# ChristianSteger/HORAYZON

Measured on AMD Instinct MI355X. Metric: grid_cells_per_s (horizon_gridded, 360 azimuths, 3601^2 SRTM-like tile), higher is better.
Workload: dtype f32

## Files before the change

horayzon_amd/csrc/hz_api.hip:

```cpp
#include "hz_internal.h"
#include "hz_horisun_plan.h"
#include "hz_horisun_coarse_plan.h"
#include <cmath>
#include <cstring>
#include <cstdlib>
#include <string>
#include <vector>
#include <limits>
#include <mutex>
#include <utility>
#include <thread>
#include <atomic>

namespace hz {

static thread_local std::string g_error;

int set_error(int code, const char *fmt, ...) {
    char buf[1024];
    va_list ap;
    va_start(ap, fmt);
    vsnprintf(buf, sizeof(buf), fmt, ap);
    va_end(ap);
    g_error = buf;
// ... 644 lines not shown
        const int rb = row_begin + k * chunk_rows, re = std::min(rb + chunk_rows, row_end);
        const void *src = (k & 1) ? tmp_hori2 : tmp_hori;
        Ev &e = evs[ev_of[(size_t)k]];
        char *dst = reinterpret_cast<char *>(hori_row0 + (size_t)rb * dim_in_1 * azim_num);
        const size_t bytes = (size_t)(re - rb) * row_bytes;
        std::vector<size_t> cuts;
        if (!pinner.planned.empty()) cuts = pinner.cuts_for(dst, bytes);
        cuts.push_back(bytes);
        if (hipStreamWaitEvent(st_copy, e.c, 0) != hipSuccess)
            return set_error(HZ_ERR_HIP, "copy of the horizon chunk failed: %s", hipGetErrorString(hipGetLastError()));
        size_t from = 0;
        for (size_t to : cuts) {
            if (to > from && hipMemcpyAsync(dst + from, static_cast<const char *>(src) + from, to - from, hipMemcpyDeviceToHost, st_copy) != hipSuccess)
                return set_error(HZ_ERR_HIP, "copy of the horizon chunk failed: %s", hipGetErrorString(hipGetLastError()));
            from = to;
        }
        if (hipEventRecord(e.d, st_copy) != hipSuccess)
            return set_error(HZ_ERR_HIP, "copy of the horizon chunk failed: %s", hipGetErrorString(hipGetLastError()));
        return HZ_OK;
    };
    auto fail = [&](int code) { (void)hipStreamSynchronize(st); if (st_copy) (void)hipStreamSynchronize(st_copy); free_events(); return code; };
    int n_chunk = 0;
    unsigned long long left_cells = 0, left_again = 0;
    float ms_left = 0.0f;
    for (int rb = row_begin; rb < row_end; rb += chunk_rows, n_chunk++) {
        const int re = std::min(rb + chunk_rows, row_end);
        float *hori_chunk;
        if (stream_out) hori_chunk = (float *)((n_chunk & 1) ? tmp_hori2 : tmp_hori);
        else if (skip_hori || to_planes) hori_chunk = (float *)tmp_hori;
        else hori_chunk = d_hori.dev + (size_t)(rb - row_begin) * dim_in_1 * azim_num;
        a.hori = hori_chunk - (size_t)rb * dim_in_1 * azim_num;
        a.row_begin = rb; a.row_end = re;
        if (use_near) {
            NearArgs na;
            na.vec_norm = norm0; na.vec_north = north0; na.mask = mask0;
            na.azim_sin = d_as.dev; na.azim_cos = d_ac.dev;
            na.offset_0 = offset_0; na.offset_1 = offset_1; na.dim_in_1 = dim_in_1; na.row_begin = rb; na.row_end = re;
            na.azim_num = azim_num; na.elev_num = tb.elev_num;
            na.ray_org_elev = ray_org_elev; na.hori_acc = tb.hori_acc; na.low = tb.low; na.up = tb.up;
            na.reasons = near_reasons;
            na.ignore_bad_map = near_opt < 0 ? 1 : 0;
            if ((rc = near_prepass(sc, na, st, &ms_near))) return fail(rc);
            a.near_idx = na.near_idx; a.near_r = na.near_r;
        }
        {
            Ev e;
// ... 81 lines not shown
                const size_t cc = (size_t)(re - rb) * dim_in_1, c0 = plane_cell0 + (size_t)(rb - row_begin) * dim_in_1;
                if (planes_on_dev) rc = hori_to_planes_launch(hori_chunk, cc, azim_num, hori_planes, plane_stride, c0, st);
                else {
                    rc = hori_to_planes_launch(hori_chunk, cc, azim_num, (float *)tmp_planes, cc, 0, st);
                    if (!rc && hipMemcpy2DAsync(hori_planes + c0, plane_stride * sizeof(float), tmp_planes, cc * sizeof(float),
                                                cc * sizeof(float), (size_t)azim_num, hipMemcpyDeviceToHost, st) != hipSuccess)
                        rc = set_error(HZ_ERR_HIP, "copy of the horizon planes failed: %s", hipGetErrorString(hipGetLastError()));
                }
            }
            if (!rc && stream_out && n_chunk >= 1) rc = copy_out(n_chunk - 1);
            if (rc) return fail(rc);
            unsigned long long c[HZ_CNT_N];
            if (hipMemcpyAsync(c, cnt_dev, sizeof(c), hipMemcpyDeviceToHost, st) != hipSuccess ||
                hipStreamSynchronize(st) != hipSuccess)
                return fail(set_error(HZ_ERR_HIP, "horizon kernel failed: %s", hipGetErrorString(hipGetLastError())));
            float m1 = 0.0f, m2 = 0.0f;
            (void)hipEventElapsedTime(&m1, e.a, e.b);
            (void)hipEventElapsedTime(&m2, e.b, e.c);
            ms += m1; ms_svf += m2;
            if (evs.back().l) { float m3 = 0.0f; (void)hipEventElapsedTime(&m3, evs.back().l, e.b); ms_left += m3; }
            for (int k = 0; k < 16; k++) cnt[k] += c[k];
            left_cells += c[28]; left_again += c[29];
            n_verified += c[21];
            if (a.count_work && opts && opts->verbose >= 3) {
                const unsigned long long t0 = ~c[20];
                fprintf(stderr, "hz xcd spans [ms] rows %d..%d:", rb, re);
                for (int x = 0; x < 8; x++) fprintf(stderr, " %.1f", c[12 + x] ? (double)(c[12 + x] - t0) * 1.0e-5 : 0.0);
                fprintf(stderr, "\n");
            }
        }
    }
    Timer t_d2h; t_d2h.start();
    if (stream_out) {
        rc = copy_out(n_chunk - 1);
        const hipError_t se = hipStreamSynchronize(st_copy);
        pinner.finish();
        if (!rc && se != hipSuccess) rc = set_error(HZ_ERR_HIP, "copy of the horizon failed: %s", hipGetErrorString(se));
        if (rc) { free_events(); return rc; }
    }
    free_events();
    HZ_HIP(hipGetLastError());
    if ((rc = d_hori.finish(st))) return rc;
    if ((rc = d_svf.finish(st))) return rc;
    if ((rc = d_vsf.finish(st))) return rc;
    if ((rc = d_open.finish(st))) return rc;
    HZ_HIP(hipStreamSynchronize(st));
    const double d2h_s = t_d2h.stop();

    if (stats) {
        stats->num_rays += cnt[0]; stats->guard_events += cnt[1];
        stats->nodes_visited += cnt[2]; stats->tris_tested += cnt[3]; stats->num_cells += cnt[4];
        stats->wave_node_iters += cnt[5]; stats->wave_leaf_iters += cnt[6]; stats->wave_refills += cnt[7];
        stats->t_h2d_s += h2d_s; stats->t_kernel_s += (double)ms * 1e-3; stats->t_svf_s += (double)ms_svf * 1e-3;
        stats->t_d2h_s += d2h_s;
        stats->t_total_s += t_total.stop();
        stats->elev_num = tb.elev_num; stats->bvh_height = sc->hdr.height; stats->scene_bytes = sc->hdr.total_bytes;
        stats->stack_fallbacks += (uint64_t)fallbacks; stats->stack_redo_blocks += redo_blocks; stats->left_redo_groups += redo_groups;
        stats->rays_shortened += cnt[9]; stats->near_violations += cnt[10] + n_mon_violations; stats->t_near_s += (double)ms_near * 1e-3;
        stats->guard_cells += cnt[11]; stats->near_verified += n_verified;
        stats->t_left_s += (double)ms_left * 1e-3; stats->left_cells += left_cells; stats->left_again += left_again;
        stats->scratch_bytes = (uint64_t)((use_near ? sc->near_bytes : 0) + (n_left_launches > 0 ? sc->left_bytes : 0) + tmp_bytes);
        stats->height_field = height_field ? 1 : 0; stats->near_used = use_near ? 1 : 0;
    }
    if (near_reasons) print_near_reasons(near_reasons);
    if (opts && opts->verbose)
        print_reference_report(sc, alg, cnt[4], cnt[0], slab_cells, dim_in_0, dim_in_1, azim_num, (double)ms * 1e-3,
                               !use_near && near_opt <= 0 && !height_field && !bad_map, use_near && bad_map);
    return HZ_OK;
}

static int locations_run(const Scene *sc, const float *coords, const float *vec_norm, const float *vec_north,
                         float *hori_buffer, float *hori_dist_buffer, int num_loc, int azim_num,
                         float dist_search, float hori_acc, const char *ray_algorithm, float elev_ang_low_lim,
                         const float *ray_org_elev, int hori_dist_out, const hz_opts *opts, hz_stats *stats) {
    int alg = 1;
    int rc = parse_alg(ray_algorithm, &alg);
    if (rc) return rc;
    if (hori_dist_out && alg == 2)
        return set_error(HZ_ERR_ARG, "horizon detection algorithm 'guess_constant' not implemented for horizon "
                                     "distance computation");
    if (!coords || !vec_norm || !vec_north || !ray_org_elev || !hori_buffer) return set_error(HZ_ERR_ARG, "NULL argument");
    if (hori_dist_out && !hori_dist_buffer) return set_error(HZ_ERR_ARG, "hori_dist_buffer is NULL");
    if (num_loc <= 0 || azim_num <= 0) return set_error(HZ_ERR_ARG, "num_loc and azim_num must be positive");
    if (!(hori_acc > 0.0f) || hori_acc > 10.0f) return set_error(HZ_ERR_ARG, "limit of hori_acc (10 degree) is exceeded");
    HZ_HIP(hipSetDevice(sc->device));
    std::lock_guard<std::mutex> run_lock(sc->run_mu);
    hipStream_t st = sc->stream;
// ... 545 lines not shown
    const size_t bytes = (n ? n : 1) * 4;
    HZ_HIP(hipMalloc(&di, bytes)); HZ_HIP(hipMalloc(&dout, bytes)); HZ_HIP(hipMalloc(&tmp, scan_temp_elems(n) * 4 + 16));
    HZ_HIP(hipMemcpy(di, in, n * 4, hipMemcpyHostToDevice));
    rc = exclusive_scan_u32((const uint32_t *)di, (uint32_t *)dout, n, (uint32_t *)tmp, st);
    if (!rc) {
        HZ_HIP(hipStreamSynchronize(st));
        HZ_HIP(hipMemcpy(out, dout, n * 4, hipMemcpyDeviceToHost));
    }
    (void)hipFree(di); (void)hipFree(dout); (void)hipFree(tmp);
    return rc;
}

int hz_debug_valu_peak(int device, int packed, int waves_per_simd, double *winst_per_s_per_simd,
                       double *clock_ghz, int *simds) {
    int rc = select_device(device);
    if (rc) return rc;
    return bench_valu_peak(packed, waves_per_simd, winst_per_s_per_simd, clock_ghz, simds);
}

int hz_debug_set(const char *key, int value) {
    if (!key) return hz::set_error(HZ_ERR_ARG, "hz_debug_set: null key");
    if (!strcmp(key, "shadow_fast_cap")) hz::g_shadow_fast_cap.store(value < 0 ? HZ_SHADOW_FAST_CAP_DEFAULT : value, std::memory_order_relaxed);
    else if (!strcmp(key, "topo_wide")) hz::g_topo_wide.store(value != 0, std::memory_order_relaxed);
    else if (!strcmp(key, "accum_chunk")) hz::g_accum_chunk.store(value < 0 ? 0 : value, std::memory_order_relaxed);
    else if (!strcmp(key, "coarse_tile")) hz::g_coarse_tile.store(value < 0 ? 0 : value, std::memory_order_relaxed);
    else if (!strcmp(key, "horisun_chunk")) hz::g_horisun_chunk.store(value < 0 ? 0 : value, std::memory_order_relaxed);
    else if (!strcmp(key, "horisun_coarse_tile")) hz::g_horisun_coarse_tile.store(value < 0 ? 0 : value, std::memory_order_relaxed);
    else if (!strcmp(key, "horisun_coarse_route")) hz::g_horisun_coarse_route.store(value < 0 ? -1 : (value == 1 ? 1 : 0), std::memory_order_relaxed);
    else if (!strcmp(key, "planes_chunk")) g_planes_chunk.store(value < 0 ? 0 : value, std::memory_order_relaxed);
    else return hz::set_error(HZ_ERR_ARG, "hz_debug_set: unknown key '%s'", key);
    return HZ_OK;
}

int hz_debug_inst_rate(int device, int op, double *cycles_per_inst) {
    int rc = select_device(device);
    if (rc) return rc;
    return bench_inst_rate(op, cycles_per_inst);
}

int hz_debug_copy_peak(int device, size_t bytes, double *gbs) {
    int rc = select_device(device);
    if (rc) return rc;
    return bench_copy_peak(bytes, gbs);
}

static int slope_api(int which, const float *x, const float *y, const float *z, int len_0, int len_1,
// ... 1085 lines not shown
```

horayzon_amd/csrc/hz_common.h:

```cpp
#pragma once
#include <stdint.h>
#include <hip/hip_runtime.h>

#define HZ_BLOB_MAGIC 0x485a4c42u
#define HZ_BLOB_VERSION 10u
#define HZ_WAVE 64

struct BlobHeader {
    uint32_t magic, version;
    int32_t d0, d1;
    int32_t n_quads, n_tin, n_prims, n_nodes;
    int32_t height, n_top;
    float center[3];
    float pad;
    float lo[3], hi[3];
    uint32_t reserved0[2];
    uint64_t off_verts, off_nodes, off_prims, total_bytes;
    uint64_t off_anc;
    int32_t anc_levels;
    int32_t n_prim_slots;
    uint32_t flags;
    uint32_t n_flipped;
    uint64_t off_bad;
    int32_t bad_nb;
// ... 291 lines not shown
__device__ __forceinline__ void hz_load_node_lds(const float4 *q, float4 &n0, uint4 &n1) {
    const unsigned addr = (unsigned)(size_t)reinterpret_cast<const __attribute__((address_space(3))) char *>(
        (const __attribute__((address_space(3))) float4 *)q);
    asm volatile("ds_read_b128 %0, %2\n\t"
                 "ds_read_b128 %1, %2 offset:16\n\t"
                 "s_waitcnt lgkmcnt(0)"
                 : "=&v"(n0), "=&v"(n1)
                 : "v"(addr)
                 : "memory");
}

__device__ __forceinline__ void hz_load_prim(const Prim *q, float4 &q0, float4 &q1, float4 &q2) {
    asm volatile("global_load_dwordx4 %0, %3, off\n\t"
                 "global_load_dwordx4 %1, %3, off offset:16\n\t"
                 "global_load_dwordx4 %2, %3, off offset:32\n\t"
                 "s_waitcnt vmcnt(0)"
                 : "=&v"(q0), "=&v"(q1), "=&v"(q2)
                 : "v"(q)
                 : "memory");
}

struct TravCounters { unsigned nodes, tris, w_nodes, w_leaves;
};
struct TravState { int node, sp, pf, pm, lq0, lq1; };

__device__ __forceinline__ void hz_trav_reset(TravState &t) {
    t.node = 0; t.sp = 0; t.pf = 0; t.pm = 0; t.lq0 = HZ_EMPTY; t.lq1 = HZ_EMPTY;
}

__device__ __forceinline__ int hz_entry_pack(int pf, int pm) {
    return (int)((unsigned)pf | (((unsigned)pm >> 1) & 3u) | (((unsigned)pm & 8u) << 27));
}
__device__ __forceinline__ void hz_entry_unpack(int e, int &pf, int &pm) {
    pm = (int)((((unsigned)e & 3u) << 1) | (((unsigned)e >> 27) & 8u));
    pf = (int)((unsigned)e & 0xbffffffcu);
}

#define HZ_WAVE_TICK(c, lane_) do { const unsigned long long m_ = __ballot(1); if ((lane_) == __ffsll((long long)m_) - 1) (c)++; } while (0)

template <int TPB, bool COUNT, int QLEN = 2, bool NODELET = false, bool LEVELSTACK = true>
__device__ __forceinline__ int hz_trace(const Node *__restrict__ nodes, const Prim *__restrict__ prims,
                                        const float4 *top, int ntop, int *stack, int tid,
                                        float ox, float oy, float oz, float dx, float dy, float dz, float tfar,
                                        float tfar_box, const RayBox &rb, TravState &t, int regroup, int leaf_bias,
                                        TravCounters &cnt, int stack_cap, bool &overflow) {
    const int lane = tid & 63;
    int node = t.node, sp = t.sp, pf = t.pf, pm = t.pm, lq0 = t.lq0, lq1 = t.lq1;
    const int n_entry = __popcll(__ballot(1));
#define HZ_POP() do { \
        if (LEVELSTACK) { \
            if (pm == 0) { const bool ne = sp > 0; sp = ne ? sp - 1 : 0; const int pv = stack[sp * TPB + tid]; \
                           hz_entry_unpack(ne ? pv : 0, pf, pm); } \
            const int slot_ = __builtin_ctz((unsigned)pm | 16u); \
            node = (pm != 0) ? pf + slot_ : HZ_EMPTY; pm &= pm - 1; \
        } else { \
            node = HZ_STACK_AT(sa + (unsigned)(TPB * 4)); sa -= (unsigned)(TPB * 4); \
        } } while (0)
typedef __attribute__((address_space(3))) int hz_lds_int;
#define HZ_STACK_AT(addr) (*reinterpret_cast<hz_lds_int *>((size_t)(addr)))
#define HZ_SAVE() do { if (!LEVELSTACK) sp = (int)(sa - sa0) / (TPB * 4) + 1; \
                       t.node = node; t.sp = sp; t.pf = pf; t.pm = pm; t.lq0 = lq0; t.lq1 = lq1; } while (0)
    const unsigned sa0 = (unsigned)(size_t)reinterpret_cast<hz_lds_int *>(
                             (__attribute__((address_space(3))) char *)reinterpret_cast<char *>(stack)) + (unsigned)tid * 4u;
    unsigned sa = sa0 + (unsigned)(sp - 1) * (unsigned)(TPB * 4);
    const unsigned sa_cap = sa0 + (unsigned)(stack_cap - 5) * (unsigned)(TPB * 4);
    if (!LEVELSTACK) HZ_STACK_AT(sa0) = HZ_EMPTY;
    unsigned sa_hi = 0u;
    const int n_leave = max(min(regroup, n_entry), 1);
// ... 43 lines not shown
                        if (pm != 0) { stack[sp * TPB + tid] = hz_entry_pack(pf, pm); sp++; }
                        pf = first; pm = h;
                    }
                    HZ_POP();
                } else {
                    int m0, m1, m2, m3;
                    hz_node_hit_masks(nr, rb, tfar_box, n1, m0, m1, m2, m3);
                    sa_hi = max(sa_hi, sa);
                    sa = min(sa, sa_cap);
                    const unsigned S = (unsigned)(TPB * 4);
                    const int pv = HZ_STACK_AT(sa + S);
                    const unsigned a0 = (unsigned)m0 & S, a1 = (unsigned)m1 & S, a2 = (unsigned)m2 & S, a3 = (unsigned)m3 & S;
                    const unsigned o32 = a3 | a2, o321 = o32 | a1, o3210 = o321 | a0;
#define HZ_SEL(m, x, y) (((m) & (x)) | (~(m) & (y)))
                    int next = HZ_SEL(m3, first + 3, pv);
                    HZ_STACK_AT(sa + 2u * S) = next; sa += a2 & a3;   next = HZ_SEL(m2, first + 2, next);
                    HZ_STACK_AT(sa + 2u * S) = next; sa += a1 & o32;  next = HZ_SEL(m1, first + 1, next);
                    HZ_STACK_AT(sa + 2u * S) = next; sa += a0 & o321; next = HZ_SEL(m0, first, next);
#undef HZ_SEL
                    node = next; sa = sa + o3210 - S;
                }
            }
        } else {
            if (can_leaf) {
                float4 q0, q1, q2;
                hz_load_prim(prims + HZ_LEAF_ID(lq0), q0, q1, q2);
                if (COUNT) { cnt.tris += (q2.y == q2.y) ? 2 : 1; HZ_WAVE_TICK(cnt.w_leaves, lane); }
                const bool hit = hz_quad_hit(ox, oy, oz, dx, dy, dz, tfar, q0.x, q0.y, q0.z, q0.w, q1.x, q1.y, q1.z, q1.w,
                                             q2.x, q2.y, q2.z, q2.w, q2.y == q2.y);
                if (hit) { lq0 = HZ_LEAF_ID(lq0); node = HZ_EMPTY; }
                else { lq0 = lq1; lq1 = HZ_EMPTY; }
            }
        }
        top_of_iteration();
    }
    if (!LEVELSTACK && sa_hi > sa_cap) overflow = true;
    const bool blocked = lq0 >= 0 && lq0 != HZ_EMPTY;
    const int res = blocked ? 1 : ((HZ_IS_NODE(node) || lq0 < 0) ? 2 : 0);
    if (blocked) lq0 = (int)((unsigned)lq0 | 0x80000000u);
    HZ_SAVE();
    return res;
#undef HZ_POP
#undef HZ_SAVE
#undef HZ_STACK_AT
}

// ... 43 lines not shown
```

horayzon_amd/csrc/hz_horizon.hip:

```cpp
#include "hz_search.h"
#include <vector>

namespace hz {

#ifndef HZ_TPB
#define HZ_TPB 256
#endif
#define HZ_WPB (HZ_TPB / 64)
#ifndef HZ_QLEN
#define HZ_QLEN 2
#endif

struct HorizonParams {
    SceneView sv;
    Tables tb;
    const float *vec_norm, *vec_north;
    const uint8_t *mask;
    float *hori;
    int offset_0, offset_1, dim_in_1;
    int row_begin, row_end;
    TileMap tm;
    float dist, hori_fill, ray_org_elev;
    float dist_box, neg_tau;
    int top_nodes, regroup, stack_bytes, leaf_bias, stage_bytes, hit_cache, stack_cap;
// ... 5 lines not shown
    unsigned verify_mask;
    unsigned long long *counters;
    const int *tile_list;
    int n_list;
    int *redo_list;
    int left_min, left_mode;
    unsigned left_in_base;
    unsigned left_out_base, left_out_cap;
    unsigned *left_rec, *left_in_ctl, *left_out_ctl;
    const unsigned *left_perm;
    int persist;
    unsigned *queue;
};

__device__ __forceinline__ void hz_left_write(unsigned *w, unsigned cert, unsigned k, unsigned flags,
                                                        unsigned ind, unsigned prev, unsigned pazim, unsigned count, float lim_up, float lim_low,
                                                        float elev_samp, float ev, unsigned cache, float st0, float st1, float st2) {
    w[0] = cert;
    w[1] = k; w[2] = flags; w[3] = ind; w[4] = prev; w[5] = pazim; w[6] = count;
    w[7] = __float_as_uint(lim_up); w[8] = __float_as_uint(lim_low); w[9] = __float_as_uint(elev_samp); w[10] = __float_as_uint(ev);
    w[11] = cache; w[12] = __float_as_uint(st0); w[13] = __float_as_uint(st1); w[14] = __float_as_uint(st2); w[15] = 0u;
}

template <int ALG, bool COUNT, bool STAGE, bool NODELET, bool LEVELSTACK, bool LEFT = false>
#ifndef HZ_WG_PER_CU
#define HZ_WG_PER_CU 5
#endif
__global__ __launch_bounds__(HZ_TPB, (COUNT ? 4 : HZ_WG_PER_CU) * (4 / HZ_WPB)) void k_horizon(HorizonParams p_arg) {
    typedef const __attribute__((address_space(4))) HorizonParams *hz_kparams;
    hz_kparams pk = (hz_kparams)__builtin_amdgcn_kernarg_segment_ptr();
#if defined(__HIP_DEVICE_COMPILE__)
#define HZ_LOAD_PARAMS(dst) dst = *pk
#else
#define HZ_LOAD_PARAMS(dst) dst = p_arg
#endif
    HorizonParams p;
    HZ_LOAD_PARAMS(p);
    extern __shared__ __attribute__((aligned(16))) unsigned char smem[];
    int *stack = reinterpret_cast<int *>(smem + p.pre_bytes);
    const float4 *top = reinterpret_cast<const float4 *>(smem + p.pre_bytes + p.stack_bytes);
    const int tid = threadIdx.x;
    const int ntop = p.top_nodes;
    if (NODELET && ntop > 0) {
        float4 *dst = reinterpret_cast<float4 *>(smem + p.pre_bytes + p.stack_bytes);
        const float4 *src = reinterpret_cast<const float4 *>(p.sv.nodes);
        for (int i = tid; i < ntop * 2; i += HZ_TPB) dst[i] = src[i];
        __syncthreads();
// ... 98 lines not shown
            done = true;
        } else {
            const float norm_x = p.vec_norm[3 * cell], norm_y = p.vec_norm[3 * cell + 1], norm_z = p.vec_norm[3 * cell + 2];
            const float north_x = p.vec_north[3 * cell], north_y = p.vec_north[3 * cell + 1], north_z = p.vec_north[3 * cell + 2];
            const float *v = p.sv.verts + 3 * ((size_t)(i + p.offset_0) * p.sv.d1 + (size_t)(j + p.offset_1));
            ox = v[0] + norm_x * p.ray_org_elev;
            oy = v[1] + norm_y * p.ray_org_elev;
            oz = v[2] + norm_z * p.ray_org_elev;
            r01 = north_x; r02 = norm_x;
            r11 = north_y; r12 = norm_y;
            r21 = north_z; r22 = norm_z;
        }
    }
#define HZ_OC(ocx, ocy, ocz) float ocx, ocy, ocz; { float ax_ = ox, ay_ = oy, az_ = oz; \
        asm volatile("" : "+v"(ax_), "+v"(ay_), "+v"(az_)); \
        ocx = ax_ - p.sv.cx; ocy = ay_ - p.sv.cy; ocz = az_ - p.sv.cz; }
    const float tfar = p.dist;

    Search s;
    s.k = 0; s.phase = PH_NEWAZ; s.ind = 0; s.prev = 0; s.pazim = 0; s.count = 0;
    s.lim_up = 0; s.lim_low = 0; s.elev_samp = 0; s.ev = 0;
    unsigned rays = 0, guards = 0, w_adv = 0;
    TravCounters tc; tc.nodes = 0; tc.tris = 0; tc.w_nodes = 0; tc.w_leaves = 0;
    const unsigned cells_cnt = (in_dom && !done && !LEFT) ? 1u : 0u;
    bool ray_active = false, last_hit = false;
    float dx = 0, dy = 0, dz = 1;
    RayBox rb = hz_raybox(0, 0, 0, 0, 0, 1);
    TravState ts; hz_trav_reset(ts);
    int cache = 0;
    bool second = false;
    bool overflow = false;
    unsigned shortened = 0;
    unsigned w_verified = 0, w_violations = 0;
    bool verifying = false, first_result = false, want_v = false;
    float tn = 0.0f;
    bool had_guard = false;
    if (LEFT && !done) {
        s.k = (int)rec[1]; s.phase = (int)(rec[2] & 0xffu); s.ind = (int)rec[3]; s.prev = (int)rec[4]; s.pazim = (int)rec[5]; s.count = (int)rec[6];
        s.lim_up = __uint_as_float(rec[7]); s.lim_low = __uint_as_float(rec[8]); s.elev_samp = __uint_as_float(rec[9]); s.ev = __uint_as_float(rec[10]);
        cache = (int)rec[11];
        last_hit = (rec[2] & 0x100u) != 0u;
        had_guard = (rec[2] & 0x400u) != 0u;
        if (STAGE) { out.stage[0] = __uint_as_float(rec[12]); out.stage[out.stride] = __uint_as_float(rec[13]); out.stage[2 * out.stride] = __uint_as_float(rec[14]); }
        if (rec[2] & 0x200u) {
            const float ec = t.elev_cos[s.ind], es = t.elev_sin[s.ind];
            const float rx = ec * t.azim_sin[s.k], ry = ec * t.azim_cos[s.k], rz = es;
// ... 59 lines not shown
                dx = (r00 * rx + r01 * ry) + r02 * rz;
                dy = (r10 * rx + r11 * ry) + r12 * rz;
                dz = (r20 * rx + r21 * ry) + r22 * rz;
                    tn = (s.ind >= near_i) ? near_rad : p.neg_tau;
                if (COUNT && tn > 0.0f) shortened++;
                if (COUNT) want_v = p.verify_near && tn > 0.0f && (((rays + cert) & p.verify_mask) == 0u);
                HZ_OC(ocx, ocy, ocz)
                rb = hz_raybox(ocx + tn * dx, ocy + tn * dy, ocz + tn * dz, dx, dy, dz);
                hz_trav_reset(ts);
                second = p.hit_cache && (cache != 0) && (s.ind <= s.pazim) && (s.k > 0);
                if (second) {
                    ts.node = cache;
                    if (!LEVELSTACK) { ts.sp = 1; stack[HZ_TPB + tid] = 0; second = false; }
                }
                ray_active = true;
                rays++;
            } else {
                done = true;
            }
        }
        bool start_v = false, viol = false;
        if (ray_active) {
            int r;
            r = hz_trace<HZ_TPB, COUNT, HZ_QLEN, NODELET, LEVELSTACK>(p.sv.nodes, p.sv.prims, top, ntop, stack, tid, ox, oy, oz,
                                                 dx, dy, dz, tfar, p.dist_box, rb, ts, p.regroup, p.leaf_bias, tc, p.stack_cap, overflow);
            if (r == 0 && second) {
                second = false; hz_trav_reset(ts);
            } else if (COUNT && want_v && r != 2) {
                want_v = false; verifying = true; first_result = (r == 1); start_v = true;
                HZ_OC(ocx, ocy, ocz)
                rb = hz_raybox(ocx + p.neg_tau * dx, ocy + p.neg_tau * dy, ocz + p.neg_tau * dz, dx, dy, dz);
                hz_trav_reset(ts);
            } else if (r != 2) {
                if (COUNT && verifying) { viol = ((r == 1) != first_result); verifying = false; }
                ray_active = false; last_hit = (r == 1);
                if (r == 1) cache = p.sv.anc[HZ_LEAF_ID(ts.lq0)];
            }
        }
        if (COUNT) {
            w_verified += (unsigned)__popcll(__ballot(start_v));
            w_violations += (unsigned)__popcll(__ballot(viol));
        }
    }
    unsigned long long r = rays, g = guards, nc = tc.nodes, tcn = tc.tris, cc = cells_cnt;
    unsigned long long wn = tc.w_nodes, wl = tc.w_leaves, wa = w_adv;
    for (int off = 32; off > 0; off >>= 1) {
        r += __shfl_xor(r, off); g += __shfl_xor(g, off); cc += __shfl_xor(cc, off);
        if (COUNT) {
            nc += __shfl_xor(nc, off); tcn += __shfl_xor(tcn, off);
            wn += __shfl_xor(wn, off); wl += __shfl_xor(wl, off); wa += __shfl_xor(wa, off);
        }
    }
    const bool wave_overflowed = !LEVELSTACK && __ballot(overflow) != 0ull;
    if (wave_overflowed) {
        if (lane == 0) {
            const unsigned long long slot = atomicAdd(&p.counters[LEFT ? 30 : 8], 1ull);
            if (slot < (unsigned long long)HZ_REDO_CAP) p.redo_list[(LEFT ? HZ_REDO_CAP : 0) + (int)slot] = blk;
        }
    } else {
    const int guard_cells = __popcll(__ballot(guards != 0u && !(LEFT && had_guard)));
    if (lane == 0) {
        if (r) atomicAdd(&p.counters[0], r);
        if (g) { atomicAdd(&p.counters[1], g); atomicAdd(&p.counters[11], (unsigned long long)guard_cells); }
        if (cc) atomicAdd(&p.counters[4], cc);
        if (COUNT) {
            atomicAdd(&p.counters[2], nc); atomicAdd(&p.counters[3], tcn);
            atomicAdd(&p.counters[5], wn); atomicAdd(&p.counters[6], wl); atomicAdd(&p.counters[7], wa);
        }
    }
    if (COUNT) {
        if (lane == 0) {
            const unsigned xcc = __builtin_amdgcn_s_getreg((3 << 11) | 20) & 7u;
            atomicMax(&p.counters[12 + xcc], (unsigned long long)wall_clock64());
            atomicMax(&p.counters[20], ~t_start);
        }
    }
    if (COUNT) {
        unsigned long long sh = shortened;
        for (int off = 32; off > 0; off >>= 1) sh += __shfl_xor(sh, off);
        if (lane == 0) {
            if (sh) atomicAdd(&p.counters[9], sh);
            if (w_violations) atomicAdd(&p.counters[10], (unsigned long long)w_violations);
            if (w_verified) atomicAdd(&p.counters[21], (unsigned long long)w_verified);
        }
    }
    }
    if (!p.persist) break;
  }
}

static long long resident_workgroups(const void *func, size_t lds) {
    struct Key { const void *f; size_t lds; int dev; long long n; };
    static std::mutex mu;
    static std::vector<Key> cache;
    int dev = 0;
    if (hipGetDevice(&dev) != hipSuccess) { (void)hipGetLastError(); return 0; }
    std::lock_guard<std::mutex> lock(mu);
    for (const Key &k : cache) if (k.f == func && k.lds == lds && k.dev == dev) return k.n;
    int per_cu = 0;
    hipDeviceProp_t prop;
    long long n = 0;
    if (hipOccupancyMaxActiveBlocksPerMultiprocessor(&per_cu, func, HZ_TPB, lds) == hipSuccess && per_cu > 0 &&
        hipGetDeviceProperties(&prop, dev) == hipSuccess && prop.multiProcessorCount > 0)
        n = (long long)per_cu * prop.multiProcessorCount;
    else (void)hipGetLastError();
    cache.push_back(Key{func, lds, dev, n});
    return n;
}

template <int ALG, bool COUNT, bool STAGE, bool NODELET, bool LEVELSTACK>
static int launch_one(const HorizonParams &p_in, int grid, size_t lds, int persist_grid, hipStream_t st) {
    const void *func = reinterpret_cast<const void *>(k_horizon<ALG, COUNT, STAGE, NODELET, LEVELSTACK>);
    HZ_HIP(hipFuncSetAttribute(func, hipFuncAttributeMaxDynamicSharedMemorySize, (int)lds));
    HorizonParams p = p_in;
    if (p.persist) {
        const long long resident = persist_grid > 0 ? (long long)persist_grid : resident_workgroups(func, lds);
        if (resident <= 0 || (long long)grid <= resident) p.persist = 0;
        else {
            grid = (int)resident;
            HZ_HIP(hipMemsetAsync(p.queue, 0, 8 * sizeof(unsigned), st));
        }
    }
    hipLaunchKernelGGL((k_horizon<ALG, COUNT, STAGE, NODELET, LEVELSTACK>), dim3(grid), dim3(HZ_TPB), lds, st, p);
    HZ_HIP(hipGetLastError());
    return HZ_OK;
}

template <int ALG, bool STAGE, bool LS>
static int launch_left(const HorizonParams &p, size_t lds, int persist_grid, hipStream_t st) {
    const void *func = reinterpret_cast<const void *>(k_horizon<ALG, false, STAGE, false, LS, true>);
    HZ_HIP(hipFuncSetAttribute(func, hipFuncAttributeMaxDynamicSharedMemorySize, (int)lds));
    long long grid = p.tile_list ? (long long)((p.n_list + HZ_WPB - 1) / HZ_WPB)
                                 : (persist_grid > 0 ? (long long)persist_grid : resident_workgroups(func, lds));
    if (grid <= 0) grid = 1024;
    hipLaunchKernelGGL((k_horizon<ALG, false, STAGE, false, LS, true>), dim3((unsigned)grid), dim3(HZ_TPB), lds, st, p);
    HZ_HIP(hipGetLastError());
    return HZ_OK;
}

__device__ __forceinline__ unsigned hz_spread16(unsigned v) {
    v &= 0xffffu; v = (v | (v << 8)) & 0x00ff00ffu; v = (v | (v << 4)) & 0x0f0f0f0fu; v = (v | (v << 2)) & 0x33333333u; v = (v | (v << 1)) & 0x55555555u;
    return v;
}
__global__ __launch_bounds__(256) void k_left_keys(const unsigned *__restrict__ rec, unsigned cap, unsigned *__restrict__ ctl, unsigned dim_in_1,
                                                   unsigned azim_num, int morton_shift, int class_shift, unsigned *__restrict__ keys,
                                                   unsigned *__restrict__ vals) {
    const unsigned idx = blockIdx.x * 256u + threadIdx.x;
    const unsigned cnt = min(ctl[0], cap);
    bool valid = false;
    unsigned key = 0x00ffffffu;
    if (idx < cnt) {
        const unsigned c = rec[(size_t)idx * HZ_LEFT_WORDS];
        if (c != 0xffffffffu) {
            valid = true;
            const unsigned k = rec[(size_t)idx * HZ_LEFT_WORDS + 1];
            const unsigned r = min(azim_num > k ? azim_num - k : 0u, 511u);
            const unsigned di = c / dim_in_1, j = c - di * dim_in_1;
            const unsigned m = ((hz_spread16(di >> 4) << 1) | hz_spread16(j >> 4)) >> morton_shift;
// ... 3 lines not shown
    if (idx < cap) { keys[idx] = key; vals[idx] = idx; }
    const unsigned long long vm = __ballot(valid);
    if ((threadIdx.x & 63) == 0 && vm != 0ull) atomicAdd(&ctl[1], (unsigned)__popcll(vm));
}

int left_sort(const HorizonArgs &a, int r, hipStream_t st) {
    const unsigned cap = a.left_cap[r];
    if (cap == 0 || a.left_rec == nullptr || a.left_sort == nullptr) return HZ_OK;
    unsigned *ctl = reinterpret_cast<unsigned *>(a.counters + HZ_CNT_LEFT) + 16 * r;
    const int rows = a.row_end - a.row_begin;
    int bits = 0;
    while ((1 << bits) < std::max((rows + 15) / 16, (a.dim_in_1 + 15) / 16)) bits++;
    const int shift = std::max(0, 2 * bits - 15);
    uint32_t *ka = a.left_sort, *va = ka + a.left_cap_max, *kb = va + a.left_cap_max, *vb = kb + a.left_cap_max, *tmp = vb + a.left_cap_max;
    hipLaunchKernelGGL(k_left_keys, dim3((cap + 255u) / 256u), dim3(256), 0, st, a.left_rec + (size_t)a.left_base[r] * HZ_LEFT_WORDS, cap, ctl,
                       (unsigned)a.dim_in_1, (unsigned)a.azim_num, shift, a.left_key_shift, ka, va);
    HZ_HIP(hipGetLastError());
    return radix_sort_pairs_u32(ka, va, kb, vb, cap, tmp, st, 3);
}

template <int ALG>
static int launch_alg(const HorizonParams &p, int grid, size_t lds, bool count, bool level_stack, int pg, hipStream_t st) {
    const bool stage = p.stage_bytes != 0;
    if (p.left_mode) {
        if (level_stack) return stage ? launch_left<ALG, true, true>(p, lds, pg, st) : launch_left<ALG, false, true>(p, lds, pg, st);
        return stage ? launch_left<ALG, true, false>(p, lds, pg, st) : launch_left<ALG, false, false>(p, lds, pg, st);
    }
    if (ALG == ALG_GUESS && !count && p.top_nodes > 0) {
        if (!level_stack) return stage ? launch_one<ALG_GUESS, false, true, true, false>(p, grid, lds, pg, st)
                                       : launch_one<ALG_GUESS, false, false, true, false>(p, grid, lds, pg, st);
        return stage ? launch_one<ALG_GUESS, false, true, true, true>(p, grid, lds, pg, st)
                     : launch_one<ALG_GUESS, false, false, true, true>(p, grid, lds, pg, st);
    }
    if (level_stack) {
        if (count) return stage ? launch_one<ALG, true, true, false, true>(p, grid, lds, pg, st) : launch_one<ALG, true, false, false, true>(p, grid, lds, pg, st);
        return stage ? launch_one<ALG, false, true, false, true>(p, grid, lds, pg, st) : launch_one<ALG, false, false, false, true>(p, grid, lds, pg, st);
    }
    if (count) return stage ? launch_one<ALG, true, true, false, false>(p, grid, lds, pg, st) : launch_one<ALG, true, false, false, false>(p, grid, lds, pg, st);
    return stage ? launch_one<ALG, false, true, false, false>(p, grid, lds, pg, st) : launch_one<ALG, false, false, false, false>(p, grid, lds, pg, st);
}

int horizon_num_blocks(const HorizonArgs &a) {
    const int rows = a.row_end - a.row_begin;
    if (rows <= 0 || a.dim_in_1 <= 0) return 0;
    const TileMap tm = make_tile_map((rows + 15) / 16, (a.dim_in_1 + 15) / 16);
    return tm.per_xcd * 8 * 4;
}

int horizon_launch(const Scene *sc, const HorizonArgs &a, hipStream_t st, int *used_level_stack) {
    HorizonParams p;
    p.sv = scene_view(sc);
    p.tb.azim_sin = a.azim_sin; p.tb.azim_cos = a.azim_cos;
    p.tb.elev_ang = a.elev_ang; p.tb.elev_sin = a.elev_sin; p.tb.elev_cos = a.elev_cos; p.tb.mid_idx = a.mid_idx;
    p.tb.azim_num = a.azim_num; p.tb.elev_num = a.elev_num;
    p.tb.hori_acc = a.hori_acc; p.tb.low = a.low; p.tb.up = a.up;
    p.tb.step = (double)a.hori_acc / 5.0;
    p.vec_norm = a.vec_norm; p.vec_north = a.vec_north;
    p.mask = a.mask; p.hori = a.hori;
    p.offset_0 = a.offset_0; p.offset_1 = a.offset_1; p.dim_in_1 = a.dim_in_1;
// ... 390 lines not shown
```

horayzon_amd/csrc/hz_internal.h:

```cpp
#pragma once
#include <hip/hip_runtime.h>
#include <algorithm>
#include <chrono>
#include <cstdarg>
#include <cstdio>
#include <cstdlib>
#include "../../include/horayzon_hip.h"
#include "hz_common.h"
#include <atomic>
#include <mutex>

#define HZ_MAX_TOP_NODES 2047
#define HZ_MAX_STACK 40
#ifndef HZ_ANC_LEVELS
#define HZ_ANC_LEVELS 4
#endif

namespace hz {

int set_error(int code, const char *fmt, ...);

#define HZ_SHADOW_FAST_CAP_DEFAULT 19
extern std::atomic<int> g_shadow_fast_cap;
extern std::atomic<int> g_topo_wide;
extern std::atomic<int> g_accum_chunk;
extern std::atomic<int> g_coarse_tile;
extern std::atomic<int> g_horisun_chunk;
extern std::atomic<int> g_horisun_coarse_tile;
extern std::atomic<int> g_horisun_coarse_route;

#define HZ_HIP(expr)                                                                      \
    do {                                                                                  \
        hipError_t e_ = (expr);                                                           \
        if (e_ != hipSuccess)                                                             \
            return ::hz::set_error(HZ_ERR_HIP, "%s failed: %s (%s:%d)", #expr,            \
                                   hipGetErrorString(e_), __FILE__, __LINE__);            \
    } while (0)

struct Timer {
    std::chrono::high_resolution_clock::time_point t0;
    void start() { t0 = std::chrono::high_resolution_clock::now(); }
    double stop() const {
        return std::chrono::duration<double>(std::chrono::high_resolution_clock::now() - t0).count();
    }
};

// ... 253 lines not shown
```

horayzon_amd/horizon.py:

```python
import ctypes as C

import numpy as np

from . import _lib
from . import _validate as V
from ._lib import Scene, hz_opts, hz_stats, hz_topo_out, ptr

TOPO_NAMES = ("svf", "vsf", "openness")
LAYOUTS = ("cell_major", "azim_major")
last_stats = None
schedule_overrides = {}


def _check_f32(a, ndim, name):
    if not isinstance(a, np.ndarray):
        raise TypeError("Argument '%s' has incorrect type (expected numpy.ndarray, got %s)"
                        % (name, type(a).__name__))
    if a.ndim != ndim:
        raise ValueError("Buffer has wrong number of dimensions (expected %d, got %d)" % (ndim, a.ndim))
    if a.dtype != np.float32:
        raise ValueError("Buffer dtype mismatch, expected 'float32_t' but got '%s'" % a.dtype.name)


def check_layout(layout):
# ... 34 lines not shown
    _lib.check((L.hz_hori_to_planes if to_planes else L.hz_hori_from_planes)(ptr(hori), y, x, a, ptr(out), device))
    return out


def to_azim_major(hori, *, device=0):
    return _convert(hori, True, device)


def to_cell_major(planes, *, device=0):
    return _convert(planes, False, device)


def horizon_gridded(vert_grid, dem_dim_0, dem_dim_1, vec_norm, vec_north,
                    offset_0, offset_1, dist_search, azim_num=360, hori_acc=0.25,
                    ray_algorithm="guess_constant", geom_type="grid",
                    vert_simp=np.array([0.0, 0.0, 0.0, 0.0], dtype=np.float32),
                    num_vert_simp=1,
                    tri_ind_simp=np.array([0, 0, 0, 0], dtype=np.int32),
                    num_tri_simp=1, elev_ang_low_lim=-15.0, mask=None,
                    hori_fill=0.0, ray_org_elev=0.01, *, device=0, verbose=False,
                    scene=None, svf_vec_tilt=None, svf_only=False, rows=None, count_work=False, devices=None,
                    topo=None, topo_vec_tilt=None, topo_only=False, layout="cell_major",
                    _top_nodes=-1, _regroup=-1, _hit_cache=True, _chunk_rows=0, _near_skip=True, _level_stack=False,
                    _verify_near=False, _left_min=0, _persist_grid=0):
    global last_stats
    _check_f32(vert_grid, 1, "vert_grid")
    _check_f32(vec_norm, 3, "vec_norm")
    _check_f32(vec_north, 3, "vec_north")
    _check_f32(vert_simp, 1, "vert_simp")
    if not isinstance(tri_ind_simp, np.ndarray) or tri_ind_simp.ndim != 1 or tri_ind_simp.dtype != np.int32:
        raise ValueError("Buffer dtype mismatch, expected 'int32_t' for tri_ind_simp")
    if mask is not None and (not isinstance(mask, np.ndarray) or mask.ndim != 2):
        raise ValueError("Buffer has wrong number of dimensions (expected 2) for mask")

    if mask is None:
        mask = np.ones(vec_norm.shape[:2], dtype=np.uint8)
    V.run((
        (ValueError, "inconsistency between input arguments vert_grid, dem_dim_0 and dem_dim_1",
         lambda: not V.fits_grid(len(vert_grid), dem_dim_0, dem_dim_1)),
        (ValueError, "inconsistency between input arguments dem_dim_0, dem_dim_1, offset_0, offset_1 and vec_norm",
         lambda: not V.window_inside(offset_0, offset_1, vec_norm.shape, dem_dim_0, dem_dim_1)),
        (ValueError, V.MSG_NORTH, lambda: not V.same_leading_shape((vec_norm, vec_north), 3, 3)),
        (ValueError, V.MSG_ALG, lambda: ray_algorithm not in V.ALGORITHMS),
        (ValueError, V.MSG_GEOM, lambda: geom_type not in V.GEOMETRIES),
        (ValueError, "inconsistency between input arguments vert_simp and num_vert_simp", lambda: len(vert_simp) < num_vert_simp * 3),
        (ValueError, "inconsistency between input arguments tri_ind_simp and num_tri_simp", lambda: len(tri_ind_simp) < num_tri_simp * 3),
        (ValueError, "triangle indices of simplified outer domain exceed number of vertices",
# ... 25 lines not shown
    ))

    planes = check_layout(layout)
    if planes and (svf_only or topo_only):
        raise ValueError("'svf_only' / 'topo_only' cannot be combined with layout=\"azim_major\": there is no horizon to lay out")

    vert_grid = np.ascontiguousarray(vert_grid)
    vec_norm = np.ascontiguousarray(vec_norm)
    vec_north = np.ascontiguousarray(vec_north)
    vert_simp = np.ascontiguousarray(vert_simp)
    tri_ind_simp = np.ascontiguousarray(tri_ind_simp)
    mask = np.ascontiguousarray(mask)

    dim_in_0, dim_in_1 = vec_norm.shape[0], vec_norm.shape[1]
    if svf_only and svf_vec_tilt is None:
        raise ValueError("'svf_only' needs 'svf_vec_tilt'")
    hori_shape = (azim_num, dim_in_0, dim_in_1) if planes else (dim_in_0, dim_in_1, azim_num)
    hori_buffer = None if (svf_only or topo_only) else np.empty(hori_shape, dtype=np.float32)
    if rows is not None and hori_buffer is not None:
        hori_buffer.fill(np.nan)

    opts = hz_opts()
    opts.device = device
    opts.verbose = int(bool(verbose))
    opts.top_nodes = _top_nodes
    opts.regroup = _regroup
    opts.no_hit_cache = 0 if _hit_cache else 1
    opts.chunk_rows = _chunk_rows
    opts.no_near_skip = -1 if _near_skip == "force" else (0 if _near_skip else 1)
    opts.level_stack = int(_level_stack)
    opts.left_min = int(_left_min or schedule_overrides.get("left_min", 0))
    opts.persist_grid = int(_persist_grid or schedule_overrides.get("persist_grid", 0))
    opts.left_cap_test = int(schedule_overrides.get("left_cap_test", 0))
    opts.left_tune = int(schedule_overrides.get("left_tune", 0))
    n_verify = int(_verify_near)
    if n_verify < 0 or n_verify != _verify_near:
        raise ValueError("_verify_near must be a non-negative integer (or a bool)")
    opts.verify_near = n_verify
    opts.skip_hori = 1 if (svf_only or topo_only) else 0
    opts.count_work = int(bool(count_work))
    if rows is not None:
        if len(rows) != 2 or not (0 <= int(rows[0]) < int(rows[1]) <= dim_in_0):
            raise ValueError("'rows' must be (begin, end) with 0 <= begin < end <= %d" % dim_in_0)
        opts.row_begin, opts.row_end = int(rows[0]), int(rows[1])
    svf = None
    if svf_vec_tilt is not None:
        _check_f32(svf_vec_tilt, 3, "svf_vec_tilt")
# ... 184 lines not shown
```

Baseline: 9.922 million.

## Lend idle lanes to neighbour's second queued leaf test via DPP swap

```diff
diff --git a/horayzon_amd/csrc/hz_api.hip b/horayzon_amd/csrc/hz_api.hip
--- a/horayzon_amd/csrc/hz_api.hip
+++ b/horayzon_amd/csrc/hz_api.hip
@@ -690,6 +690,7 @@
     auto fail = [&](int code) { (void)hipStreamSynchronize(st); if (st_copy) (void)hipStreamSynchronize(st_copy); free_events(); return code; };
     int n_chunk = 0;
     unsigned long long left_cells = 0, left_again = 0;
+    unsigned long long lend_tests = 0, lend_unhelped = 0;
     float ms_left = 0.0f;
     for (int rb = row_begin; rb < row_end; rb += chunk_rows, n_chunk++) {
         const int re = std::min(rb + chunk_rows, row_end);
@@ -817,6 +818,7 @@
             for (int k = 0; k < 16; k++) cnt[k] += c[k];
             left_cells += c[28]; left_again += c[29];
             n_verified += c[21];
+            lend_tests += c[22]; lend_unhelped += c[23];
             if (a.count_work && opts && opts->verbose >= 3) {
                 const unsigned long long t0 = ~c[20];
                 fprintf(stderr, "hz xcd spans [ms] rows %d..%d:", rb, re);
@@ -858,6 +860,10 @@
         stats->height_field = height_field ? 1 : 0; stats->near_used = use_near ? 1 : 0;
     }
     if (near_reasons) print_near_reasons(near_reasons);
+    if (a.count_work && opts && opts->verbose >= 2 && lend_tests + lend_unhelped > 0)
+        fprintf(stderr, "hz leaf lending: %llu lent leaf tests, %llu leaf-step lanes with a second leaf and no helper (a = %.3f); "
+                        "wave leaf steps %llu, wave node steps %llu, triangles tested %llu\n", lend_tests, lend_unhelped,
+                (lend_tests + lend_unhelped) ? (double)lend_tests / (double)(lend_tests + lend_unhelped) : 0.0, cnt[6], cnt[5], cnt[3]);
     if (opts && opts->verbose)
         print_reference_report(sc, alg, cnt[4], cnt[0], slab_cells, dim_in_0, dim_in_1, azim_num, (double)ms * 1e-3,
                                !use_near && near_opt <= 0 && !height_field && !bad_map, use_near && bad_map);
@@ -1449,6 +1455,7 @@
     if (!key) return hz::set_error(HZ_ERR_ARG, "hz_debug_set: null key");
     if (!strcmp(key, "shadow_fast_cap")) hz::g_shadow_fast_cap.store(value < 0 ? HZ_SHADOW_FAST_CAP_DEFAULT : value, std::memory_order_relaxed);
     else if (!strcmp(key, "topo_wide")) hz::g_topo_wide.store(value != 0, std::memory_order_relaxed);
+    else if (!strcmp(key, "leaf_lend")) hz::g_leaf_lend.store(value != 0, std::memory_order_relaxed);
     else if (!strcmp(key, "accum_chunk")) hz::g_accum_chunk.store(value < 0 ? 0 : value, std::memory_order_relaxed);
     else if (!strcmp(key, "coarse_tile")) hz::g_coarse_tile.store(value < 0 ? 0 : value, std::memory_order_relaxed);
     else if (!strcmp(key, "horisun_chunk")) hz::g_horisun_chunk.store(value < 0 ? 0 : value, std::memory_order_relaxed);
diff --git a/horayzon_amd/csrc/hz_common.h b/horayzon_amd/csrc/hz_common.h
--- a/horayzon_amd/csrc/hz_common.h
+++ b/horayzon_amd/csrc/hz_common.h
@@ -337,6 +337,7 @@
 
 struct TravCounters { unsigned nodes, tris, w_nodes, w_leaves;
 };
+struct LendCounters { unsigned lent, unhelped; };
 struct TravState { int node, sp, pf, pm, lq0, lq1; };
 
 __device__ __forceinline__ void hz_trav_reset(TravState &t) {
@@ -353,12 +354,12 @@
 
 #define HZ_WAVE_TICK(c, lane_) do { const unsigned long long m_ = __ballot(1); if ((lane_) == __ffsll((long long)m_) - 1) (c)++; } while (0)
 
-template <int TPB, bool COUNT, int QLEN = 2, bool NODELET = false, bool LEVELSTACK = true>
+template <int TPB, bool COUNT, int QLEN = 2, bool NODELET = false, bool LEVELSTACK = true, bool LEND = false>
 __device__ __forceinline__ int hz_trace(const Node *__restrict__ nodes, const Prim *__restrict__ prims,
                                         const float4 *top, int ntop, int *stack, int tid,
                                         float ox, float oy, float oz, float dx, float dy, float dz, float tfar,
                                         float tfar_box, const RayBox &rb, TravState &t, int regroup, int leaf_bias,
-                                        TravCounters &cnt, int stack_cap, bool &overflow) {
+                                        TravCounters &cnt, int stack_cap, bool &overflow, LendCounters *lcnt = nullptr) {
     const int lane = tid & 63;
     int node = t.node, sp = t.sp, pf = t.pf, pm = t.pm, lq0 = t.lq0, lq1 = t.lq1;
     const int n_entry = __popcll(__ballot(1));
@@ -448,6 +449,41 @@
                 }
             }
         } else {
+            if (LEND && !LEVELSTACK) {
+                static_assert(HZ_EMPTY > 1, "the idle word must be neither a queued link (negative) nor HZ_EMPTY");
+                int p_w = 0, lf;
+                float rox, roy, roz, rdx, rdy, rdz;
+#define HZ_DPP_SEL(d, x) "v_cndmask_b32_dpp %[" d "], %[" x "], %[" x "], vcc quad_perm:[1,0,3,2] row_mask:0xf bank_mask:0xf bound_ctrl:1\n\t"
+                asm volatile("s_mov_b64 vcc, %[m]\n\t"
+                             "v_cndmask_b32_e32 %[lf], 1, %[lq1], vcc\n\t"
+                             HZ_DPP_SEL("rox", "ox") HZ_DPP_SEL("roy", "oy") HZ_DPP_SEL("roz", "oz")
+                             HZ_DPP_SEL("rdx", "dx") HZ_DPP_SEL("rdy", "dy") HZ_DPP_SEL("rdz", "dz")
+                             "v_mov_b32_dpp %[pw], %[lf] quad_perm:[1,0,3,2] row_mask:0xf bank_mask:0xf\n\t"
+                             "v_cndmask_b32_e32 %[lf], %[pw], %[lq0], vcc"
+                             : [pw] "+&v"(p_w), [lf] "=&v"(lf), [rox] "=&v"(rox), [roy] "=&v"(roy), [roz] "=&v"(roz),
+                               [rdx] "=&v"(rdx), [rdy] "=&v"(rdy), [rdz] "=&v"(rdz)
+                             : [m] "s"(m_leaf), [lq0] "v"(lq0), [lq1] "v"(lq1), [ox] "v"(ox), [oy] "v"(oy), [oz] "v"(oz),
+                               [dx] "v"(dx), [dy] "v"(dy), [dz] "v"(dz)
+                             : "vcc");
+#undef HZ_DPP_SEL
+                const bool helper = !can_leaf && p_w < 0;
+                const bool helped = can_leaf && lq1 < 0 && p_w == 1;
+                if (COUNT && lcnt && can_leaf && lq1 < 0 && p_w != 1) lcnt->unhelped++;
+                if (can_leaf || helper) {
+                    float4 q0, q1, q2;
+                    hz_load_prim(prims + HZ_LEAF_ID(lf), q0, q1, q2);
+                    if (COUNT) { cnt.tris += (q2.y == q2.y) ? 2 : 1; HZ_WAVE_TICK(cnt.w_leaves, lane); if (lcnt && helper) lcnt->lent++; }
+                    const bool hit = hz_quad_hit(rox, roy, roz, rdx, rdy, rdz, tfar, q0.x, q0.y, q0.z, q0.w, q1.x, q1.y, q1.z, q1.w,
+                                                 q2.x, q2.y, q2.z, q2.w, q2.y == q2.y);
+                    const int p_hit = __builtin_amdgcn_update_dpp(0, hit ? 1 : 0, 0xB1, 0xF, 0xF, true);
+                    const bool lent_hit = helped && p_hit != 0;
+                    const bool any = hit || lent_hit;
+                    const int n_lq0 = any ? HZ_LEAF_ID(hit ? lq0 : lq1) : (helped ? HZ_EMPTY : lq1);
+                    node = (can_leaf && any) ? HZ_EMPTY : node;
+                    lq1 = (can_leaf && !any) ? HZ_EMPTY : lq1;
+                    lq0 = can_leaf ? n_lq0 : lq0;
+                }
+            } else
             if (can_leaf) {
                 float4 q0, q1, q2;
                 hz_load_prim(prims + HZ_LEAF_ID(lq0), q0, q1, q2);
diff --git a/horayzon_amd/csrc/hz_horizon.hip b/horayzon_amd/csrc/hz_horizon.hip
--- a/horayzon_amd/csrc/hz_horizon.hip
+++ b/horayzon_amd/csrc/hz_horizon.hip
@@ -51,7 +51,7 @@
     w[11] = cache; w[12] = __float_as_uint(st0); w[13] = __float_as_uint(st1); w[14] = __float_as_uint(st2); w[15] = 0u;
 }
 
-template <int ALG, bool COUNT, bool STAGE, bool NODELET, bool LEVELSTACK, bool LEFT = false>
+template <int ALG, bool COUNT, bool STAGE, bool NODELET, bool LEVELSTACK, bool LEFT = false, bool LEND = false>
 #ifndef HZ_WG_PER_CU
 #define HZ_WG_PER_CU 5
 #endif
@@ -196,6 +196,7 @@
     s.lim_up = 0; s.lim_low = 0; s.elev_samp = 0; s.ev = 0;
     unsigned rays = 0, guards = 0, w_adv = 0;
     TravCounters tc; tc.nodes = 0; tc.tris = 0; tc.w_nodes = 0; tc.w_leaves = 0;
+    LendCounters lc; lc.lent = 0; lc.unhelped = 0;
     const unsigned cells_cnt = (in_dom && !done && !LEFT) ? 1u : 0u;
     bool ray_active = false, last_hit = false;
     float dx = 0, dy = 0, dz = 1;
@@ -301,8 +302,8 @@
         bool start_v = false, viol = false;
         if (ray_active) {
             int r;
-            r = hz_trace<HZ_TPB, COUNT, HZ_QLEN, NODELET, LEVELSTACK>(p.sv.nodes, p.sv.prims, top, ntop, stack, tid, ox, oy, oz,
-                                                 dx, dy, dz, tfar, p.dist_box, rb, ts, p.regroup, p.leaf_bias, tc, p.stack_cap, overflow);
+            r = hz_trace<HZ_TPB, COUNT, HZ_QLEN, NODELET, LEVELSTACK, LEND>(p.sv.nodes, p.sv.prims, top, ntop, stack, tid, ox, oy, oz,
+                                                 dx, dy, dz, tfar, p.dist_box, rb, ts, p.regroup, p.leaf_bias, tc, p.stack_cap, overflow, &lc);
             if (r == 0 && second) {
                 second = false; hz_trav_reset(ts);
             } else if (COUNT && want_v && r != 2) {
@@ -323,11 +324,13 @@
     }
     unsigned long long r = rays, g = guards, nc = tc.nodes, tcn = tc.tris, cc = cells_cnt;
     unsigned long long wn = tc.w_nodes, wl = tc.w_leaves, wa = w_adv;
+    unsigned long long ln = lc.lent, un = lc.unhelped;
     for (int off = 32; off > 0; off >>= 1) {
         r += __shfl_xor(r, off); g += __shfl_xor(g, off); cc += __shfl_xor(cc, off);
         if (COUNT) {
             nc += __shfl_xor(nc, off); tcn += __shfl_xor(tcn, off);
             wn += __shfl_xor(wn, off); wl += __shfl_xor(wl, off); wa += __shfl_xor(wa, off);
+            if (LEND) { ln += __shfl_xor(ln, off); un += __shfl_xor(un, off); }
         }
     }
     const bool wave_overflowed = !LEVELSTACK && __ballot(overflow) != 0ull;
@@ -345,6 +348,7 @@
         if (COUNT) {
             atomicAdd(&p.counters[2], nc); atomicAdd(&p.counters[3], tcn);
             atomicAdd(&p.counters[5], wn); atomicAdd(&p.counters[6], wl); atomicAdd(&p.counters[7], wa);
+            if (LEND) { atomicAdd(&p.counters[22], ln); atomicAdd(&p.counters[23], un); }
         }
     }
     if (COUNT) {
@@ -367,6 +371,8 @@
     if (!p.persist) break;
   }
 }
+
+std::atomic<int> g_leaf_lend{1};
 
 static long long resident_workgroups(const void *func, size_t lds) {
     struct Key { const void *f; size_t lds; int dev; long long n; };
@@ -387,9 +393,9 @@
     return n;
 }
 
-template <int ALG, bool COUNT, bool STAGE, bool NODELET, bool LEVELSTACK>
+template <int ALG, bool COUNT, bool STAGE, bool NODELET, bool LEVELSTACK, bool LEND = false>
 static int launch_one(const HorizonParams &p_in, int grid, size_t lds, int persist_grid, hipStream_t st) {
-    const void *func = reinterpret_cast<const void *>(k_horizon<ALG, COUNT, STAGE, NODELET, LEVELSTACK>);
+    const void *func = reinterpret_cast<const void *>(k_horizon<ALG, COUNT, STAGE, NODELET, LEVELSTACK, false, LEND>);
     HZ_HIP(hipFuncSetAttribute(func, hipFuncAttributeMaxDynamicSharedMemorySize, (int)lds));
     HorizonParams p = p_in;
     if (p.persist) {
@@ -400,19 +406,19 @@
             HZ_HIP(hipMemsetAsync(p.queue, 0, 8 * sizeof(unsigned), st));
         }
     }
-    hipLaunchKernelGGL((k_horizon<ALG, COUNT, STAGE, NODELET, LEVELSTACK>), dim3(grid), dim3(HZ_TPB), lds, st, p);
+    hipLaunchKernelGGL((k_horizon<ALG, COUNT, STAGE, NODELET, LEVELSTACK, false, LEND>), dim3(grid), dim3(HZ_TPB), lds, st, p);
     HZ_HIP(hipGetLastError());
     return HZ_OK;
 }
 
-template <int ALG, bool STAGE, bool LS>
+template <int ALG, bool STAGE, bool LS, bool LEND = false>
 static int launch_left(const HorizonParams &p, size_t lds, int persist_grid, hipStream_t st) {
-    const void *func = reinterpret_cast<const void *>(k_horizon<ALG, false, STAGE, false, LS, true>);
+    const void *func = reinterpret_cast<const void *>(k_horizon<ALG, false, STAGE, false, LS, true, LEND>);
     HZ_HIP(hipFuncSetAttribute(func, hipFuncAttributeMaxDynamicSharedMemorySize, (int)lds));
     long long grid = p.tile_list ? (long long)((p.n_list + HZ_WPB - 1) / HZ_WPB)
                                  : (persist_grid > 0 ? (long long)persist_grid : resident_workgroups(func, lds));
     if (grid <= 0) grid = 1024;
-    hipLaunchKernelGGL((k_horizon<ALG, false, STAGE, false, LS, true>), dim3((unsigned)grid), dim3(HZ_TPB), lds, st, p);
+    hipLaunchKernelGGL((k_horizon<ALG, false, STAGE, false, LS, true, LEND>), dim3((unsigned)grid), dim3(HZ_TPB), lds, st, p);
     HZ_HIP(hipGetLastError());
     return HZ_OK;
 }
@@ -462,8 +468,10 @@
 template <int ALG>
 static int launch_alg(const HorizonParams &p, int grid, size_t lds, bool count, bool level_stack, int pg, hipStream_t st) {
     const bool stage = p.stage_bytes != 0;
+    const bool lend = !level_stack && g_leaf_lend.load(std::memory_order_relaxed) != 0;
     if (p.left_mode) {
         if (level_stack) return stage ? launch_left<ALG, true, true>(p, lds, pg, st) : launch_left<ALG, false, true>(p, lds, pg, st);
+        if (lend) return stage ? launch_left<ALG, true, false, true>(p, lds, pg, st) : launch_left<ALG, false, false, true>(p, lds, pg, st);
         return stage ? launch_left<ALG, true, false>(p, lds, pg, st) : launch_left<ALG, false, false>(p, lds, pg, st);
     }
     if (ALG == ALG_GUESS && !count && p.top_nodes > 0) {
@@ -475,6 +483,10 @@
     if (level_stack) {
         if (count) return stage ? launch_one<ALG, true, true, false, true>(p, grid, lds, pg, st) : launch_one<ALG, true, false, false, true>(p, grid, lds, pg, st);
         return stage ? launch_one<ALG, false, true, false, true>(p, grid, lds, pg, st) : launch_one<ALG, false, false, false, true>(p, grid, lds, pg, st);
+    }
+    if (lend) {
+        if (count) return stage ? launch_one<ALG, true, true, false, false, true>(p, grid, lds, pg, st) : launch_one<ALG, true, false, false, false, true>(p, grid, lds, pg, st);
+        return stage ? launch_one<ALG, false, true, false, false, true>(p, grid, lds, pg, st) : launch_one<ALG, false, false, false, false, true>(p, grid, lds, pg, st);
     }
     if (count) return stage ? launch_one<ALG, true, true, false, false>(p, grid, lds, pg, st) : launch_one<ALG, true, false, false, false>(p, grid, lds, pg, st);
     return stage ? launch_one<ALG, false, true, false, false>(p, grid, lds, pg, st) : launch_one<ALG, false, false, false, false>(p, grid, lds, pg, st);
diff --git a/horayzon_amd/csrc/hz_internal.h b/horayzon_amd/csrc/hz_internal.h
--- a/horayzon_amd/csrc/hz_internal.h
+++ b/horayzon_amd/csrc/hz_internal.h
@@ -22,6 +22,7 @@
 
 #define HZ_SHADOW_FAST_CAP_DEFAULT 19
 extern std::atomic<int> g_shadow_fast_cap;
+extern std::atomic<int> g_leaf_lend;
 extern std::atomic<int> g_topo_wide;
 extern std::atomic<int> g_accum_chunk;
 extern std::atomic<int> g_coarse_tile;
diff --git a/horayzon_amd/horizon.py b/horayzon_amd/horizon.py
--- a/horayzon_amd/horizon.py
+++ b/horayzon_amd/horizon.py
@@ -80,7 +80,7 @@
                     scene=None, svf_vec_tilt=None, svf_only=False, rows=None, count_work=False, devices=None,
                     topo=None, topo_vec_tilt=None, topo_only=False, layout="cell_major",
                     _top_nodes=-1, _regroup=-1, _hit_cache=True, _chunk_rows=0, _near_skip=True, _level_stack=False,
-                    _verify_near=False, _left_min=0, _persist_grid=0):
+                    _verify_near=False, _left_min=0, _persist_grid=0, _verbose=0):
     global last_stats
     _check_f32(vert_grid, 1, "vert_grid")
     _check_f32(vec_norm, 3, "vec_norm")
@@ -152,7 +152,7 @@
 
     opts = hz_opts()
     opts.device = device
-    opts.verbose = int(bool(verbose))
+    opts.verbose = max(int(bool(verbose)), int(_verbose))
     opts.top_nodes = _top_nodes
     opts.regroup = _regroup
     opts.no_hit_cache = 0 if _hit_cache else 1
```

After: 10.22 million (median of 6 runs). 3.0% higher.
